# jkrueger/phosphorus_mk2

Hardware: AMD Instinct MI355X
Metric: Mrays/sec (primary+secondary) (higher is better)
Workload: dtype f32; 1 GPU; Soup(100000, seed 1234) 1280x720 256 spp depth 9 pps 1, 1 emissive quad, Lambert 0.73 (BASELINE.json configs[1]); tiles=32x32, tile (tx, ty) -> rank (tx + 3 ty) % n_gpus, film_collective=none, frames_in_flight=1, hbm_bytes_per_rank=41566904552, film_finite=True

## Files before the change

### phosphorus_mk2_amd/csrc/kernels.hip

```cpp
#include "kernels.h"

#include <algorithm>
#include <cstddef>
#include <cstdlib>

namespace phx {

#define PHX_BLOCK 256
#ifndef PHX_PERM_LUT
#define PHX_PERM_LUT 1
#endif
#ifndef PHX_COUNT
#define PHX_COUNT 0
#endif
#ifndef PHX_SHADE_TIMING
#define PHX_SHADE_TIMING 0
#endif
#ifndef PHX_SHADE_PREFETCH
#define PHX_SHADE_PREFETCH 2
#endif

__device__ __forceinline__ uint32_t f2u(float f) { return __float_as_uint(f); }
__device__ __forceinline__ float u2f(uint32_t u) { return __uint_as_float(u); }

#ifndef PHX_SHADE_BLOCK_D
#define PHX_SHADE_BLOCK_D 1024
#endif
#ifndef PHX_SHADE_BLOCK_G
#define PHX_SHADE_BLOCK_G 512
#endif
#ifndef PHX_SHADE_WAVES_G
#define PHX_SHADE_WAVES_G 4
#endif
template <int SHADE_BLOCK>
__device__ __forceinline__ void block_append2(bool want_a, uint32_t* counter_a, bool want_b, uint32_t* counter_b, uint32_t* lds ,
                                              uint32_t& at_a, uint32_t& at_b, unsigned long long* probe = nullptr ) {
  static_assert(SHADE_BLOCK >= 128 && SHADE_BLOCK % 64 == 0, "block_append2: wave 0 sums queue A, wave 1 queue B");
  const uint32_t lane = __lane_id(), wave = threadIdx.x >> 6, nwaves = SHADE_BLOCK >> 6;
  const unsigned long long mask_a = __ballot(want_a), mask_b = __ballot(want_b);
  uint32_t* cnt_a = lds; uint32_t* cnt_b = lds + nwaves + 1;
  if (lane == 0) { cnt_a[wave] = (uint32_t)__popcll(mask_a); cnt_b[wave] = (uint32_t)__popcll(mask_b); }
  __syncthreads();
  if (lane == 0 && wave < 2) {
    uint32_t* cnt = wave == 0 ? cnt_a : cnt_b;
    uint32_t total = 0;
#pragma nounroll
    for (uint32_t w = 0; w < nwaves; ++w) { const uint32_t c = cnt[w]; cnt[w] = total; total += c; }
#if PHX_SHADE_TIMING
    const long long ta_ = clock64();
#endif
    cnt[nwaves] = total ? atomicAdd(wave == 0 ? counter_a : counter_b, total) : 0u;
#if PHX_SHADE_TIMING
    static_assert(offsetof(DevStats, tri_pending_lane_iters) == offsetof(DevStats, idle_lane_iters) + sizeof(unsigned long long), "probe[0] / probe[1] are DevStats::idle_lane_iters / tri_pending_lane_iters");
    if (probe) { asm volatile("s_waitcnt vmcnt(0)" ::: "memory"); atomicAdd(&probe[0], (unsigned long long)(clock64() - ta_)); atomicAdd(&probe[1], 1ull); }
#endif
  }
  __syncthreads();
  const unsigned long long below = (1ull << lane) - 1ull;
  at_a = cnt_a[nwaves] + cnt_a[wave] + (uint32_t)__popcll(mask_a & below);
  at_b = cnt_b[nwaves] + cnt_b[wave] + (uint32_t)__popcll(mask_b & below);
}

template <bool LENS>
__device__ __forceinline__ void camera_ray(const DevScene& sc, const PassBuffers& pb, uint32_t path, uint32_t sample0, v3& p, v3& w) {
  const uint32_t pix = path / pb.num_samples, s = path - pix * pb.num_samples;
  const uint32_t xy = pb.pix_xy[pix];
  const float sx = (float)(xy & 0xffffu), sy = (float)(xy >> 16);
  const float2 jit = pb.jitter[sample0 + s];
  const float ndcy = 0.5f - (-0.5f + sy) * sc.stepy;
  const float ndcx = (-0.5f + sx) * sc.stepx - 0.5f;
  v3 d(jit.x, jit.y, -1.0f);
  d.x = (ndcx + d.x * sc.stepx) * sc.ratio * sc.zoom;
  d.y = (ndcy + d.y * sc.stepy) * sc.zoom;
  const float ool = 1.0f / sqrtf(sdot(d, d));
  d = v3(d.x * ool, d.y * ool, d.z * ool);
  const float* M = sc.cam_m;
  if constexpr (LENS) {
    const uint32_t key = path_key(pb.seed, (xy >> 16) * sc.width + (xy & 0xffffu), sample0 + s);
    const float ux = draw_f32(key, DIM_LENS_U), uy = draw_f32(key, DIM_LENS_V);
    const float c2 = (float)(2.0f / M_PI), c4 = (float)(4.0f / M_PI);
    const bool x_gt_y = fabsf(ux) > fabsf(uy);
    const float r = x_gt_y ? uy : ux;
    const float theta1 = c4 * (uy / ux), theta2 = c2 - c4 * (ux / uy);
    const sincosf_t sc_t = sincosf_(x_gt_y ? theta2 : theta1);
    const float lx = (r * sc_t.c) * sc.aperture_radius, ly = (r * sc_t.s) * sc.aperture_radius;
    const float ft = fabsf(sc.focal_distance / d.z);
    d = v3(d.x * ft - lx, d.y * ft - ly, d.z * ft - 0.0f);
    const float ool2 = 1.0f / sqrtf(sdot(d, d));
    d = v3(d.x * ool2, d.y * ool2, d.z * ool2);
    { float t = lx * M[0]; t = fmaf(ly, M[4], t); t = fmaf(0.0f, M[8], t); p.x = t + M[12]; }
    { float t = lx * M[1]; t = fmaf(ly, M[5], t); t = fmaf(0.0f, M[9], t); p.y = t + M[13]; }
    { float t = lx * M[2]; t = fmaf(ly, M[6], t); t = fmaf(0.0f, M[10], t); p.z = t + M[14]; }
  } else {
  { float t = 0.0f * M[0]; t = fmaf(0.0f, M[4], t); t = fmaf(0.0f, M[8], t); p.x = t + M[12]; }
  { float t = 0.0f * M[1]; t = fmaf(0.0f, M[5], t); t = fmaf(0.0f, M[9], t); p.y = t + M[13]; }
  { float t = 0.0f * M[2]; t = fmaf(0.0f, M[6], t); t = fmaf(0.0f, M[10], t); p.z = t + M[14]; }
  }
  { float t = d.x * M[0]; t = fmaf(d.y, M[4], t); w.x = fmaf(d.z, M[8], t); }
  { float t = d.x * M[1]; t = fmaf(d.y, M[5], t); w.y = fmaf(d.z, M[9], t); }
  { float t = d.x * M[2]; t = fmaf(d.y, M[6], t); w.z = fmaf(d.z, M[10], t); }
}

__device__ __forceinline__ void zero_cursors(uint32_t* counters) {
#pragma unroll
  for (uint32_t k = 0; k < 2u * CNT_SEGS; ++k) counters[CNT_CURSOR + k * CNT_STRIDE] = 0;
}
__global__ void k_begin_pass(PassBuffers pb, uint32_t num_samples) {
  const uint32_t npaths = pb.num_pixels * num_samples;
  pb.counters[0] = npaths; pb.counters[CNT_STRIDE] = 0; pb.counters[CNT_SHADOW] = 0; pb.counters[CNT_SHADOW + CNT_STRIDE] = 0;
  zero_cursors(pb.counters);
  atomicAdd(&pb.stats->camera_samples, (unsigned long long)npaths);
}

template <int LEVELS>
struct LdsStack {
  uint2* base;
  int sp;
  __device__ __forceinline__ void push(uint32_t b, uint32_t h) { base[sp * PHX_BLOCK] = make_uint2(b, h); ++sp; }
  __device__ __forceinline__ void pop(uint32_t& b, uint32_t& h) { --sp; const uint2 e = base[sp * PHX_BLOCK]; b = e.x; h = e.y; }
  __device__ __forceinline__ bool empty() const { return sp == 0; }
};

#ifndef PHX_STEPS_PER_REFILL
#define PHX_STEPS_PER_REFILL 1
#endif
#ifndef PHX_WG_CHUNKS
#define PHX_WG_CHUNKS 16u
#endif
#ifndef PHX_XCD_SEGMENTS
#define PHX_XCD_SEGMENTS 1
#endif
#ifndef PHX_SPILL_FROM_LEVELS
#define PHX_SPILL_FROM_LEVELS 10u
#endif
#ifndef PHX_SPILL_LDS_LEVELS
#define PHX_SPILL_LDS_LEVELS 7u
#endif
#ifndef PHX_STACK_PACKED
#define PHX_STACK_PACKED 1
#endif
#ifndef PHX_PROBE_VALU
#define PHX_PROBE_VALU 0
#endif
#ifndef PHX_PROBE_VMEM
#define PHX_PROBE_VMEM 0
#endif
#ifndef PHX_PROBE_VMEM_DWORD
#define PHX_PROBE_VMEM_DWORD 0
#endif
#define PHX_UNI(x) ((uint32_t)__builtin_amdgcn_readfirstlane((int)(x)))
#ifndef PHX_TRACE_WATCHDOG
#define PHX_TRACE_WATCHDOG (1u << 22)
#endif
struct DynQueue {
  uint32_t n0, n1, c0, c1;
  uint32_t r0, r1;
  uint32_t num_waves;
  uint32_t* cursor;
};
template <int BLOCK, bool SPILL , bool PACKED >
__device__ __forceinline__ void trace_stream(const DevScene& sc, const PassBuffers& pb, int q,
                                             uint32_t* cursor , uint2* stack_base, uint8_t* stack_valid , uint32_t lds_levels,
                                             uint2* spill_base , uint32_t refill_min,
                                             const uint4* __restrict__ top , uint32_t ntop,
                                             const DynQueue dq, const uint8_t* __restrict__ perm_lut) {
  const uint32_t lane = __lane_id();
  bool active = false, any = false;
  uint32_t phase = 0;
  RayCtx r; r.o = v3(0.f); r.d = v3(0.f); r.idx = r.idy = r.idz = 0.f; r.oct_inv = 0;
  float tbest = 0.f, hu = 0.f, hv = 0.f;
  uint32_t htri = 0xffffffffu, hprim = 0, idx = 0, ng_base = 0, ng_hits = 0, path = 0;
  constexpr uint32_t TG_PENDING = 0xff00u;
  uint32_t tg_base = 0, tg = 0, tq_base = 0, tq = 0;
  int sp = 0;
  const float4* __restrict__ ro = pb.ro[q];
  const float4* __restrict__ rd = pb.rd[q];
  uint32_t dlo = 0, dhi = 0;
#if PHX_COUNT
  uint32_t cnt_lds[2] = {0, 0}, cnt_mem[2] = {0, 0}, cnt_tri[2] = {0, 0};
  uint32_t cnt_iter = 0, cnt_nb = 0, cnt_tb = 0, cnt_refill = 0;
  uint32_t cnt_idle = 0, cnt_pend = 0;
  uint32_t cnt_push[8] = {0, 0, 0, 0, 0, 0, 0, 0};
  uint32_t cnt_pairs = 0, cnt_pairs_hist[8] = {0, 0, 0, 0, 0, 0, 0, 0};
#endif
  uint32_t guard = 0;
  for (;;) {
    if (++guard > PHX_TRACE_WATCHDOG) { if (lane == 0) atomicAdd(&pb.stats->watchdog, 1ull); break; }
    const unsigned long long idle = __ballot(!active);
    if (phase < 2u && (uint32_t)__popcll(idle) >= refill_min) {
#if PHX_COUNT
      ++cnt_refill;
#endif
      const uint32_t leader = (uint32_t)__ffsll((long long)idle) - 1u;
      uint32_t hi, base;
      {
        if (dlo >= dhi) {
          const uint32_t c = phase == 0u ? dq.c0 : dq.c1, qn = phase == 0u ? dq.n0 : dq.n1;
          uint32_t got_lo = 0, got_hi = 0, st = 1;
          if (lane == leader) {
            unsigned long long* pack = reinterpret_cast<unsigned long long*>(cursor) + phase;
            uint32_t* fetching = cursor + 4 + phase; uint32_t* done = cursor + 6 + phase;
            const unsigned long long old = __hip_atomic_fetch_add(pack, (unsigned long long)c, __ATOMIC_RELAXED, __HIP_MEMORY_SCOPE_WORKGROUP);
            const uint32_t s0 = (uint32_t)old, e0 = (uint32_t)(old >> 32);
            if (s0 < e0) { got_lo = s0; got_hi = min(s0 + c, e0); st = 0; }
            else if (__hip_atomic_load(done, __ATOMIC_RELAXED, __HIP_MEMORY_SCOPE_WORKGROUP)) st = 2;
            else if (atomicCAS(fetching, 0u, 1u) == 0u) {
              __builtin_amdgcn_fence(__ATOMIC_ACQUIRE, "workgroup");
              const unsigned long long cur = __hip_atomic_load(pack, __ATOMIC_RELAXED, __HIP_MEMORY_SCOPE_WORKGROUP);
              if ((uint32_t)cur < (uint32_t)(cur >> 32)) st = 1;
              else if (__hip_atomic_load(done, __ATOMIC_RELAXED, __HIP_MEMORY_SCOPE_WORKGROUP)) st = 2;
              else {
                const uint32_t cwg = phase == 0u ? dq.r0 : dq.r1;
#if PHX_XCD_SEGMENTS
                uint32_t nb = qn, seg_end = qn, sgm = cursor[8 + phase];
                for (uint32_t tries = 0; tries < CNT_SEGS; ++tries, sgm = (sgm + 1u) & (CNT_SEGS - 1u)) {
                  const uint32_t lo_s = (uint32_t)((unsigned long long)qn * sgm / CNT_SEGS), hi_s = (uint32_t)((unsigned long long)qn * (sgm + 1u) / CNT_SEGS);
                  const uint32_t homes = (gridDim.x + CNT_SEGS - 1u - sgm) / CNT_SEGS;
                  const unsigned long long at = (unsigned long long)lo_s + (unsigned long long)homes * cwg + atomicAdd(&dq.cursor[(phase * CNT_SEGS + sgm) * CNT_STRIDE], cwg);
                  if (at < hi_s) { nb = (uint32_t)at; seg_end = hi_s; break; }
                }
                cursor[8 + phase] = sgm;
                if (nb >= seg_end) { __hip_atomic_store(done, 1u, __ATOMIC_RELAXED, __HIP_MEMORY_SCOPE_WORKGROUP); st = 2; }
                else {
                  const uint32_t end = min(nb + cwg, seg_end);
#else
                const uint32_t nb = atomicAdd(&dq.cursor[phase * CNT_SEGS * CNT_STRIDE], cwg) + gridDim.x * cwg;
                if (nb >= qn) { __hip_atomic_store(done, 1u, __ATOMIC_RELAXED, __HIP_MEMORY_SCOPE_WORKGROUP); st = 2; }
                else {
                  const uint32_t end = min(nb + cwg, qn);
#endif
                  got_lo = nb; got_hi = min(nb + c, end); st = 0;
                  __hip_atomic_store(pack, (unsigned long long)(nb + c) | ((unsigned long long)end << 32), __ATOMIC_RELAXED, __HIP_MEMORY_SCOPE_WORKGROUP);
                }
              }
              __builtin_amdgcn_fence(__ATOMIC_RELEASE, "workgroup");
              __hip_atomic_store(fetching, 0u, __ATOMIC_RELAXED, __HIP_MEMORY_SCOPE_WORKGROUP);
            }
          }
          st = (uint32_t)__builtin_amdgcn_readfirstlane((int)__shfl((int)st, (int)leader));
          if (st == 2u) {
            phase = PHX_UNI(phase + 1u);
            if (phase < 2u || __ballot(active) != 0ull) { if (phase < 2u) continue; } else break;
          } else if (st == 0u) {
            dlo = (uint32_t)__builtin_amdgcn_readfirstlane((int)__shfl((int)got_lo, (int)leader));
            dhi = (uint32_t)__builtin_amdgcn_readfirstlane((int)__shfl((int)got_hi, (int)leader));
          } else if (__ballot(active) == 0ull) { __builtin_amdgcn_s_sleep(4); continue; }
        }
        if (phase >= 2u) { hi = 0; base = 0; }
        else {
          const uint32_t take = PHX_UNI(min((uint32_t)__popcll(idle), dhi - dlo));
          base = dlo; hi = dlo + take; dlo = PHX_UNI(dlo + take);
        }
      }
      if (!active) {
        const uint32_t l5 = lane & 31u, below = (1u << l5) - 1u, ilo = (uint32_t)idle, ihi = (uint32_t)(idle >> 32);
        const uint32_t my = base + (uint32_t)__popc(ilo & below) + (uint32_t)__popc(ihi & below) + (lane >= 32u ? ((ilo >> l5) & 1u) : 0u);
        if (my < hi) {
          {
            float4 a, b;
            if (phase == 0u) { a = pb.so[my]; b = pb.sd[my]; } else { a = ro[my]; b = rd[my]; }
            r = make_ray_ctx(v3(a.x, a.y, a.z), v3(b.x, b.y, b.z));
            tbest = phase == 0u ? b.w : FLT_MAX; path = f2u(a.w);
          }
          hu = 0.f; hv = 0.f; htri = 0xffffffffu; hprim = 0; idx = my;
          ng_base = 0; ng_hits = 0x80000000u; tg = 0; tq = 0; sp = 0;
          any = phase == 0u;
          active = true;
        }
      }
      if (phase < 2u && __ballot(active) == 0ull) continue;
    }
    if (!__ballot(active)) break;
#if PHX_COUNT
    ++cnt_iter;
    cnt_idle += (uint32_t)__popcll(__ballot(!active));
#endif
    const bool node_ok = active && ng_hits > 0x00ffffffu && (any ? !(tg & TG_PENDING) : tq == 0u);
#if PHX_COUNT
    if (__ballot(node_ok)) ++cnt_nb;
    cnt_pend += (uint32_t)__popcll(__ballot(active && !node_ok && (tg & TG_PENDING)));
#endif
    if (node_ok) {
      const uint32_t bit = 31u - (uint32_t)__clz((int)ng_hits);
      const uint32_t rest = ng_hits & ~(1u << bit);
      if (rest > 0x00ffffffu) {
#if PHX_COUNT
        ++cnt_push[sp < 7 ? sp : 7];
#endif
        if (!SPILL || (uint32_t)sp < lds_levels) {
          if constexpr (PACKED) {
            reinterpret_cast<uint32_t*>(stack_base)[sp * BLOCK] = (ng_base & 0x00ffffffu) | (rest & 0xff000000u);
            stack_valid[((uint32_t)sp >> 2) * (BLOCK * 4u) + ((uint32_t)sp & 3u)] = (uint8_t)rest;
          } else stack_base[sp * BLOCK] = make_uint2(ng_base, rest);
        }
        else spill_base[(size_t)((uint32_t)sp - lds_levels) * sc.spill_stride] = make_uint2(ng_base, rest);
        ++sp;
      }
      const uint32_t slot = (bit - 24u) ^ r.oct_inv;
      const uint32_t ni = ng_base + (uint32_t)__popc(ng_hits & 0xffu & ~(0xffffffffu << slot));
      uint32_t w[16];
#if PHX_COUNT
      if (ni < ntop) ++cnt_lds[any ? 1 : 0]; else ++cnt_mem[any ? 1 : 0];
#endif
      const bool in_lds = ni < ntop;
      {
        const uint4* s4 = top + (in_lds ? ni : 0u) * (PHX_NODE_LDS_BYTES / 16u);
#pragma unroll
        for (int k = 0; k < 4; ++k) { const uint4 v = s4[k]; w[4 * k] = v.x; w[4 * k + 1] = v.y; w[4 * k + 2] = v.z; w[4 * k + 3] = v.w; }
      }
      if (!in_lds) {
        const uint4* s4 = reinterpret_cast<const uint4*>(sc.pool) + (size_t)ni * 4u;
#pragma unroll
        for (int k = 0; k < 4; ++k) { const uint4 v = s4[k]; w[4 * k] = v.x; w[4 * k + 1] = v.y; w[4 * k + 2] = v.z; w[4 * k + 3] = v.w; }
      }
#if PHX_PROBE_VMEM
      if (!in_lds) {
        const uint4* s4 = reinterpret_cast<const uint4*>(sc.pool) + (size_t)(ni ^ 1u) * 4u;
#pragma unroll
        for (int k = 0; k < PHX_PROBE_VMEM; ++k) {
#if PHX_PROBE_VMEM_DWORD
          w[2] ^= s4[k].x & (refill_min >> 31);
#else
          const uint4 v = s4[k]; w[2] ^= (v.x ^ v.y ^ v.z ^ v.w) & (refill_min >> 31);
#endif
        }
      }
#endif
#if PHX_PERM_LUT
      uint32_t hm = node_hitmask(w, sc.grid, r, tbest, [&](uint32_t m) { return (uint32_t)perm_lut[(r.oct_inv << 8) | m]; });
#else
      uint32_t hm = node_hitmask(w, sc.grid, r, tbest);
#endif
#if PHX_PROBE_VALU
      {
        float x = tbest;
#pragma unroll
        for (int k = 0; k < PHX_PROBE_VALU; ++k) x = __builtin_fmaf(x, 0.99999f, 1.0e-3f);
        hm ^= f2u(x) & (refill_min >> 31);
      }
#endif
      ng_base = w[3];
      ng_hits = hm & 0xff0000ffu;
      const uint32_t tnew = (hm >> 8) & TG_PENDING;
      if (tnew) {
        const uint32_t g = (hm & 0xffu) | tnew;
        if (!(tg & TG_PENDING)) { tg_base = w[3]; tg = g; }
        else { tq_base = w[3]; tq = g; }
      }
    }
    const bool tpend = active && (tg & TG_PENDING);
#if PHX_COUNT
    if (__ballot(tpend)) {
      ++cnt_tb;
      const uint32_t mine = active ? (uint32_t)__popc((tg >> 8) & 0xffu) + (uint32_t)__popc((tq >> 8) & 0xffu) : 0u;
      uint32_t pairs = 0;
      for (uint32_t b = 0; b < 5u; ++b) pairs += (uint32_t)__popcll(__ballot((mine >> b) & 1u)) << b;
      cnt_pairs += pairs;
      ++cnt_pairs_hist[pairs <= 8u ? 0 : pairs <= 16u ? 1 : pairs <= 24u ? 2 : pairs <= 32u ? 3 : pairs <= 48u ? 4 : pairs <= 64u ? 5 : pairs <= 96u ? 6 : 7];
    }
#endif
    if (tpend) {
      const uint32_t k = 23u - (uint32_t)__clz((int)(tg & TG_PENDING));
      tg &= ~(0x100u << k);
      const uint32_t ti = tg_base + (uint32_t)__popc(tg & 0xffu & ~(0xffffffffu << k));
      const uint4* t4 = reinterpret_cast<const uint4*>(sc.pool) + (size_t)ti * 4u;
      const uint4 t0 = t4[0], t1 = t4[1], t2 = t4[2];
      TriRec T;
      T.v0x = u2f(t0.x); T.v0y = u2f(t0.y); T.v0z = u2f(t0.z); T.e0x = u2f(t0.w);
      T.e0y = u2f(t1.x); T.e0z = u2f(t1.y); T.e1x = u2f(t1.z); T.e1y = u2f(t1.w);
      T.e1z = u2f(t2.x); T.prim = t2.y;
      float us, vs, ds;
#if PHX_COUNT
      ++cnt_tri[any ? 1 : 0];
#endif
      if (mt_intersect(T, r.o, r.d, tbest, hprim, us, vs, ds)) {
        tbest = ds; hu = us; hv = vs; htri = ti; hprim = T.prim;
        if (any) active = false;
      }
      if (!(tg & TG_PENDING) && tq != 0u) { tg_base = tq_base; tg = tq; tq = 0u; }
    }
    if (active && ng_hits <= 0x00ffffffu) {
      if (sp == 0) {
        if (!(tg & TG_PENDING)) {
          if (any) {
            const float4 cc = pb.sc[idx];
            float4 rr = pb.pr[path];
            rr.x += cc.x; rr.y += cc.y; rr.z += cc.z;
            pb.pr[path] = rr;
          } else {
            pb.hit[idx] = make_float4(tbest, hu, hv, u2f(htri));
          }
          active = false;
        }
      } else {
        --sp;
        uint2 e;
        if (!SPILL || (uint32_t)sp < lds_levels) {
          if constexpr (PACKED) {
            const uint32_t word = reinterpret_cast<uint32_t*>(stack_base)[sp * BLOCK];
            const uint32_t vb = stack_valid[((uint32_t)sp >> 2) * (BLOCK * 4u) + ((uint32_t)sp & 3u)];
            e = make_uint2(word & 0x00ffffffu, (word & 0xff000000u) | vb);
          } else e = stack_base[sp * BLOCK];
        }
        else e = spill_base[(size_t)((uint32_t)sp - lds_levels) * sc.spill_stride];
        ng_base = e.x; ng_hits = e.y;
      }
    }
  }
#if PHX_COUNT
  for (int k = 0; k < 2; ++k) {
    atomicAdd(&pb.stats->node_visits_lds[k], (unsigned long long)cnt_lds[k]);
    atomicAdd(&pb.stats->node_visits_mem[k], (unsigned long long)cnt_mem[k]);
    atomicAdd(&pb.stats->tri_tests[k], (unsigned long long)cnt_tri[k]);
  }
  for (int k = 0; k < 8; ++k) if (cnt_push[k]) atomicAdd(&pb.stats->stack_pushes[k], (unsigned long long)cnt_push[k]);
  if (lane == 0) {
    atomicAdd(&pb.stats->tri_block_execs, (unsigned long long)cnt_tb);
    atomicAdd(&pb.stats->wave_iters, (unsigned long long)cnt_iter);
    atomicAdd(&pb.stats->node_block_execs, (unsigned long long)cnt_nb);
    atomicAdd(&pb.stats->refills, (unsigned long long)cnt_refill);
    atomicAdd(&pb.stats->idle_lane_iters, (unsigned long long)cnt_idle);
    atomicAdd(&pb.stats->tri_pending_lane_iters, (unsigned long long)cnt_pend);
    atomicAdd(&pb.stats->tri_pairs_pending, (unsigned long long)cnt_pairs);
    for (int k = 0; k < 8; ++k) if (cnt_pairs_hist[k]) atomicAdd(&pb.stats->tri_pairs_hist[k], (unsigned long long)cnt_pairs_hist[k]);
  }
#endif
}

template <int BLOCK, bool SPILL = false, bool PACKED = false>
__global__ void __launch_bounds__(BLOCK, 8) k_trace(DevScene sc, PassBuffers pb, int q, int sq, int do_closest, int do_shadow, uint32_t refill_min,
                                                 uint32_t ntop, uint32_t levels, uint32_t min_chunks, uint32_t target_chunks) {
  extern __shared__ uint4 smem[];
  uint4* top = smem;
  uint2* stack = reinterpret_cast<uint2*>(smem + ntop * (PHX_NODE_LDS_BYTES / 16u));
  uint32_t* stack_words = reinterpret_cast<uint32_t*>(stack);
  uint32_t* valid_rows = stack_words + levels * BLOCK;
  uint32_t* cursor = PACKED ? valid_rows + ((levels + 3u) >> 2) * BLOCK : reinterpret_cast<uint32_t*>(stack + levels * BLOCK);
  uint8_t* perm_lut = reinterpret_cast<uint8_t*>(cursor + 12);
  const uint32_t n_closest = do_closest ? pb.counters[q * CNT_STRIDE] : 0u;
  const uint32_t n_shadow = do_shadow ? pb.counters[CNT_SHADOW + sq * CNT_STRIDE] : 0u;
  if (blockIdx.x == 0 && threadIdx.x == 0) {
    if (do_closest) { pb.counters[(q ^ 1) * CNT_STRIDE] = 0; pb.counters[CNT_SHADOW + (sq ^ 1) * CNT_STRIDE] = 0; }
    if (n_closest) atomicAdd(&pb.stats->rays_closest, (unsigned long long)n_closest);
    if (n_shadow) atomicAdd(&pb.stats->rays_shadow, (unsigned long long)n_shadow);
    if (do_closest && pb.qlen_out) { __hip_atomic_store(pb.qlen_out, n_closest, __ATOMIC_RELAXED, __HIP_MEMORY_SCOPE_SYSTEM); }
  }
  if (n_shadow == 0u && n_closest == 0u) return;
  DynQueue dq{};
  dq.n0 = n_shadow; dq.n1 = n_closest;
  dq.num_waves = gridDim.x * (BLOCK / 64);
  dq.cursor = pb.counters + CNT_CURSOR;
  auto chunk_of = [&](uint32_t n) { return min(max((n / (dq.num_waves * max(min_chunks, 1u)) + 63u) & ~63u, 64u), target_chunks * 64u); };
  dq.c0 = chunk_of(n_shadow); dq.c1 = chunk_of(n_closest);
  auto range_of = [&](uint32_t n, uint32_t c) { return c * min(max(n / (gridDim.x * c * 4u), 1u), PHX_WG_CHUNKS); };
  dq.r0 = range_of(n_shadow, dq.c0); dq.r1 = range_of(n_closest, dq.c1);
  if (threadIdx.x == 0) {
    unsigned long long* pack = reinterpret_cast<unsigned long long*>(cursor);
    for (uint32_t p = 0; p < 2u; ++p) {
      const uint32_t cwg = p == 0u ? dq.r0 : dq.r1, qn = p == 0u ? n_shadow : n_closest;
#if PHX_XCD_SEGMENTS
      const uint32_t sgm = blockIdx.x & (CNT_SEGS - 1u), kth = blockIdx.x / CNT_SEGS;
      const uint32_t lo_s = (uint32_t)((unsigned long long)qn * sgm / CNT_SEGS), hi_s = (uint32_t)((unsigned long long)qn * (sgm + 1u) / CNT_SEGS);
      const uint32_t lo = (uint32_t)min((unsigned long long)lo_s + (unsigned long long)kth * cwg, (unsigned long long)hi_s), hi = min(lo + cwg, hi_s);
      cursor[8 + p] = sgm;
#else
      const uint32_t lo = min(blockIdx.x * cwg, qn), hi = min(lo + cwg, qn);
#endif
      pack[p] = (unsigned long long)lo | ((unsigned long long)hi << 32);
      cursor[4 + p] = 0u; cursor[6 + p] = 0u;
    }
  }
  const uint4* g4 = reinterpret_cast<const uint4*>(sc.pool);
  for (uint32_t i = threadIdx.x; i < ntop * 4u; i += BLOCK) top[(i >> 2) * (PHX_NODE_LDS_BYTES / 16u) + (i & 3u)] = g4[i];
#if PHX_PERM_LUT
  for (uint32_t i = threadIdx.x; i < 2048u; i += BLOCK) perm_lut[i] = (uint8_t)perm_xor8(i & 0xffu, i >> 8);
#endif
  __syncthreads();
  if constexpr (PACKED)
    trace_stream<BLOCK, SPILL, true>(sc, pb, q, cursor, reinterpret_cast<uint2*>(stack_words + threadIdx.x), reinterpret_cast<uint8_t*>(valid_rows + threadIdx.x), levels,
                                     sc.stack_spill + (size_t)blockIdx.x * BLOCK + threadIdx.x, refill_min, top, ntop, dq, perm_lut);
  else
    trace_stream<BLOCK, SPILL, false>(sc, pb, q, cursor, stack + threadIdx.x, nullptr, levels, sc.stack_spill + (size_t)blockIdx.x * BLOCK + threadIdx.x,
                                      refill_min, top, ntop, dq, perm_lut);
}

template <bool ANY>
__global__ void __launch_bounds__(PHX_BLOCK) k_trace_rays(DevScene sc, uint32_t n, const float4* ro, const float4* rd, float4* hit) {
  extern __shared__ uint2 ray_stack[];
  const uint32_t i = blockIdx.x * PHX_BLOCK + threadIdx.x;
  if (i >= n) return;
  const float4 a = ro[i], b = rd[i];
  LdsStack<0> st{ray_stack + threadIdx.x, 0};
  Hit h;
  traverse8<ANY>(sc.pool, sc.grid, v3(a.x, a.y, a.z), v3(b.x, b.y, b.z), b.w, h, st);
  hit[i] = make_float4(h.t, h.u, h.v, u2f(h.tri == 0xffffffffu ? 0xffffffffu : sc.tris[h.tri].prim));
}

template <bool MAX>
__device__ __forceinline__ float wave_reduce_f(float x) {
#define PHX_DPP_STEP(ctrl, rows) { const float t = __builtin_bit_cast(float, __builtin_amdgcn_update_dpp(__builtin_bit_cast(int, x), __builtin_bit_cast(int, x), ctrl, rows, 0xf, false)); x = MAX ? fmaxf(x, t) : fminf(x, t); }
  PHX_DPP_STEP(0x111, 0xf) PHX_DPP_STEP(0x112, 0xf) PHX_DPP_STEP(0x114, 0xf) PHX_DPP_STEP(0x118, 0xf)
  PHX_DPP_STEP(0x142, 0xa) PHX_DPP_STEP(0x143, 0xc)
#undef PHX_DPP_STEP
  return __builtin_bit_cast(float, __builtin_amdgcn_readlane(__builtin_bit_cast(int, x), 63));
}
__device__ __forceinline__ float wave_min_f(float x) { return wave_reduce_f<false>(x); }
__device__ __forceinline__ float wave_max_f(float x) { return wave_reduce_f<true>(x); }
struct PacketBounds { float s[3], kn[3], kf[3], bmin[3], bmax[3]; };
__device__ __forceinline__ void packet_axis(PacketBounds& B, int a, float o_lo, float o_hi, float ia_lo, float ia_hi ,
                                            bool down ) {
  const float omin = wave_min_f(o_lo), omax = wave_max_f(o_hi);
  B.bmin[a] = wave_min_f(ia_lo); B.bmax[a] = wave_max_f(ia_hi);
  B.s[a] = down ? -1.0f : 1.0f;
  B.kn[a] = down ? omin : -omax;
  B.kf[a] = down ? omax : -omin;
}
typedef unsigned int phx_u4 __attribute__((ext_vector_type(4)));
typedef const __attribute__((address_space(4))) phx_u4* phx_const_u4p;
__device__ __forceinline__ uint32_t packet_node_hit8(const uint32_t* w, const SceneGrid& g, const PacketBounds& B, uint32_t oct_inv, float tmax_wave, uint32_t& valid) {
  float px, py, pz;
  node_origin_decode(w[0], w[1], g, px, py, pz, valid);
  const uint32_t e = w[2];
  const float sx = u32_as_f32((e & 0xffu) << 23), sy = u32_as_f32(((e >> 8) & 0xffu) << 23), sz = u32_as_f32(((e >> 16) & 0xffu) << 23);
  const uint32_t sh = (__lane_id() & 7u) * 8u;
  auto plane = [&](int row) { return (float)((uint32_t)((((unsigned long long)w[row + 1] << 32) | (unsigned long long)w[row]) >> sh) & 0xffu); };
  const float lox = fmaf(plane(4), sx, px), hix = fmaf(plane(10), sx, px);
  const float loy = fmaf(plane(6), sy, py), hiy = fmaf(plane(12), sy, py);
  const float loz = fmaf(plane(8), sz, pz), hiz = fmaf(plane(14), sz, pz);
  const bool nx = !(oct_inv & 4u), ny = !(oct_inv & 2u), nz = !(oct_inv & 1u);
  const float anx = fmaf(B.s[0], nx ? hix : lox, B.kn[0]), afx = fmaf(B.s[0], nx ? lox : hix, B.kf[0]);
  const float any_ = fmaf(B.s[1], ny ? hiy : loy, B.kn[1]), afy = fmaf(B.s[1], ny ? loy : hiy, B.kf[1]);
  const float anz = fmaf(B.s[2], nz ? hiz : loz, B.kn[2]), afz = fmaf(B.s[2], nz ? loz : hiz, B.kf[2]);
  const float tnx = anx * (anx >= 0.0f ? B.bmin[0] : B.bmax[0]), tfx = afx * (afx >= 0.0f ? B.bmax[0] : B.bmin[0]);
  const float tny = any_ * (any_ >= 0.0f ? B.bmin[1] : B.bmax[1]), tfy = afy * (afy >= 0.0f ? B.bmax[1] : B.bmin[1]);
  const float tnz = anz * (anz >= 0.0f ? B.bmin[2] : B.bmax[2]), tfz = afz * (afz >= 0.0f ? B.bmax[2] : B.bmin[2]);
  float tn = fmaxf(fmaxf(tnx, tny), tnz), tf = fminf(fminf(tfx, tfy), tfz);
  const float pad = 1.52587890625e-05f;
  tn = tn - fabsf(tn) * pad; tf = tf + fabsf(tf) * pad;
  const bool hit = tn <= tf && tf >= 0.0f && tn <= tmax_wave;
  return (uint32_t)__ballot(hit) & 0xffu & valid;
}

#define PHX_PRIMARY_BLOCK 256
#ifndef PHX_PRIMARY_WAVES
#define PHX_PRIMARY_WAVES 5
#endif
template <int RPL, bool LENS = false >
__global__ void __launch_bounds__(PHX_PRIMARY_BLOCK) __attribute__((amdgpu_waves_per_eu(PHX_PRIMARY_WAVES, 8))) k_trace_primary(DevScene sc, PassBuffers pb, uint32_t npaths, uint32_t sample0, int q, int sq) {
  extern __shared__ uint2 primary_lds[];
  uint2* lane_stacks = primary_lds + (PHX_PRIMARY_BLOCK / 64) * PHX_MAX_BVH_DEPTH;
  if (blockIdx.x == 0 && threadIdx.x == 0) {
    pb.counters[(q ^ 1) * CNT_STRIDE] = 0; pb.counters[CNT_SHADOW + (sq ^ 1) * CNT_STRIDE] = 0;
    atomicAdd(&pb.stats->rays_closest, (unsigned long long)npaths);
  }
  const uint32_t lane = __lane_id(), wave = threadIdx.x >> 6;
  const uint32_t base = (blockIdx.x * (PHX_PRIMARY_BLOCK / 64) + wave) * (64u * RPL);
  if (base >= npaths) return;
  uint32_t idx[RPL];
  RayCtx r[RPL];
  float tbest[RPL], hu[RPL], hv[RPL];
  uint32_t htri[RPL], hprim[RPL];
  bool mixed = false;
#pragma unroll
  for (int k = 0; k < RPL; ++k) {
    idx[k] = base + 64u * k + lane;
    v3 co, cd;
    camera_ray<LENS>(sc, pb, min(idx[k], npaths - 1u), sample0, co, cd);
    r[k] = make_ray_ctx(co, cd);
    tbest[k] = FLT_MAX; hu[k] = 0.0f; hv[k] = 0.0f; htri[k] = 0xffffffffu; hprim[k] = 0;
  }
  const uint32_t oct = PHX_UNI(r[0].oct_inv);
#pragma unroll
  for (int k = 0; k < RPL; ++k) mixed = mixed || r[k].oct_inv != oct;
  if (__ballot(mixed) != 0ull) {
#pragma unroll
    for (int k = 0; k < RPL; ++k) {
      LdsStack<0> st{lane_stacks + threadIdx.x, 0};
      Hit h;
      if constexpr (LENS) { const float chk = (r[k].o.x + r[k].o.y + r[k].o.z) + (r[k].d.x + r[k].d.y + r[k].d.z); if (!(fabsf(chk) <= FLT_MAX)) continue; }
      traverse8<false>(sc.pool, sc.grid, r[k].o, r[k].d, FLT_MAX, h, st);
      tbest[k] = h.t; hu[k] = h.u; hv[k] = h.v; htri[k] = h.tri;
    }
#if PHX_COUNT
    if (lane == 0) { atomicAdd(&pb.stats->primary_packets, 1ull); atomicAdd(&pb.stats->primary_fallbacks, 1ull); }
#endif
  } else {
    PacketBounds B;
    {
      v3 olo = r[0].o, ohi = r[0].o, ilo(fabsf(r[0].idx), fabsf(r[0].idy), fabsf(r[0].idz)), ihi = ilo;
#pragma unroll
      for (int k = 1; k < RPL; ++k) {
        olo = v3(fminf(olo.x, r[k].o.x), fminf(olo.y, r[k].o.y), fminf(olo.z, r[k].o.z)); ohi = v3(fmaxf(ohi.x, r[k].o.x), fmaxf(ohi.y, r[k].o.y), fmaxf(ohi.z, r[k].o.z));
        const v3 ia(fabsf(r[k].idx), fabsf(r[k].idy), fabsf(r[k].idz));
        ilo = v3(fminf(ilo.x, ia.x), fminf(ilo.y, ia.y), fminf(ilo.z, ia.z)); ihi = v3(fmaxf(ihi.x, ia.x), fmaxf(ihi.y, ia.y), fmaxf(ihi.z, ia.z));
      }
      packet_axis(B, 0, olo.x, ohi.x, ilo.x, ihi.x, !(oct & 4u)); packet_axis(B, 1, olo.y, ohi.y, ilo.y, ihi.y, !(oct & 2u)); packet_axis(B, 2, olo.z, ohi.z, ilo.z, ihi.z, !(oct & 1u));
    }
    float tmax_wave = FLT_MAX;
    uint32_t ng_base = 0, ng_hits = 0x80000000u;
    uint32_t sp = 0, guard = 0;
#if PHX_COUNT
    uint32_t cnt_nodes = 0, cnt_tris = 0, cnt_lanes = 0;
#endif
    uint2* stack = primary_lds + wave * PHX_MAX_BVH_DEPTH;
    for (;;) {
      if (++guard > PHX_TRACE_WATCHDOG) { if (lane == 0) atomicAdd(&pb.stats->watchdog, 1ull); break; }
      const uint32_t bit = 31u - (uint32_t)__clz((int)ng_hits);
      const uint32_t rest = ng_hits & ~(1u << bit);
      if (rest > 0x00ffffffu) { if (lane == 0) stack[sp] = make_uint2(ng_base, rest); ++sp; }
      const uint32_t slot = (bit - 24u) ^ oct;
      const uint32_t ni = PHX_UNI(ng_base + (uint32_t)__popc(ng_hits & 0xffu & ~(0xffffffffu << slot)));
      uint32_t w[16];
      {
        const phx_const_u4p s4 = (phx_const_u4p)(sc.pool) + (size_t)ni * 4u;
#pragma unroll
        for (int k = 0; k < 4; ++k) { const phx_u4 v = s4[k]; w[4 * k] = v.x; w[4 * k + 1] = v.y; w[4 * k + 2] = v.z; w[4 * k + 3] = v.w; }
      }
      uint32_t valid;
#if PHX_COUNT
      ++cnt_nodes;
#endif
      const uint32_t hit8 = packet_node_hit8(w, sc.grid, B, oct, tmax_wave, valid);
      const uint32_t imask = w[2] >> 24;
      ng_base = PHX_UNI(w[3]);
      ng_hits = PHX_UNI((perm_xor8(hit8 & imask, oct) << 24) | valid);
      uint32_t th = PHX_UNI(hit8 & ~imask);
      while (th != 0u) {
        const uint32_t k = 31u - (uint32_t)__clz((int)th);
        th &= ~(1u << k);
        const uint32_t ti = PHX_UNI(ng_base + (uint32_t)__popc(valid & ~(0xffffffffu << k)));
        const phx_const_u4p t4 = (phx_const_u4p)(sc.pool) + (size_t)ti * 4u;
        const phx_u4 t0 = t4[0], t1 = t4[1], t2 = t4[2];
        TriRec T;
        T.v0x = u2f(t0.x); T.v0y = u2f(t0.y); T.v0z = u2f(t0.z); T.e0x = u2f(t0.w);
        T.e0y = u2f(t1.x); T.e0z = u2f(t1.y); T.e1x = u2f(t1.z); T.e1y = u2f(t1.w);
        T.e1z = u2f(t2.x); T.prim = t2.y;
        bool any_better = false;
        float tworst = 0.0f;
#pragma unroll
        for (int m = 0; m < RPL; ++m) {
          float us, vs, ds;
          const bool better = mt_intersect(T, r[m].o, r[m].d, tbest[m], hprim[m], us, vs, ds);
          if (better) { tbest[m] = ds; hu[m] = us; hv[m] = vs; htri[m] = ti; hprim[m] = T.prim; }
          any_better = any_better || better;
          tworst = fmaxf(tworst, tbest[m]);
        }
#if PHX_COUNT
        ++cnt_tris; cnt_lanes += (uint32_t)__popcll(__ballot(any_better));
#endif
        if (__ballot(any_better) != 0ull) tmax_wave = wave_max_f(tworst);
      }
      if (ng_hits <= 0x00ffffffu) {
        if (sp == 0u) break;
        --sp;
        const uint2 e = stack[sp];
        ng_base = PHX_UNI(e.x); ng_hits = PHX_UNI(e.y);
      }
    }
#if PHX_COUNT
    if (lane == 0) {
      atomicAdd(&pb.stats->primary_packets, 1ull);
      atomicAdd(&pb.stats->primary_node_tests, (unsigned long long)cnt_nodes);
      atomicAdd(&pb.stats->primary_tri_tests, (unsigned long long)cnt_tris);
      atomicAdd(&pb.stats->primary_tri_lanes_hit, (unsigned long long)cnt_lanes);
    }
#endif
  }
#pragma unroll
  for (int k = 0; k < RPL; ++k)
    if (idx[k] < npaths) pb.hit[idx[k]] = make_float4(tbest[k], hu[k], hv[k], u2f(htri[k]));
}

__device__ __forceinline__ v3 shading_normal(const DevScene& sc, uint32_t elem , bool smooth, const v3& e0, const v3& e1, float u, float v) {
  if (smooth) {
    const float w = 1 - u - v;
    const float* pn = sc.elem_normals + 9 * (size_t)elem;
    const v3 n0(pn[0], pn[1], pn[2]), n1(pn[3], pn[4], pn[5]), n2(pn[6], pn[7], pn[8]);
    return normalize_inplace(w * n0 + u * n1 + v * n2);
  }
  return normalize_inplace(cross(e0, e1));
}
struct VertexNormals { v3 n0, n1, n2; };
__device__ __forceinline__ VertexNormals request_vertex_normals(const DevScene& sc, uint32_t elem) {
  VertexNormals N{v3(0.0f), v3(0.0f), v3(0.0f)};
  if (sc.elem_normals) {
    const float* pn = sc.elem_normals + 9 * (size_t)elem;
    N.n0 = v3(pn[0], pn[1], pn[2]); N.n1 = v3(pn[3], pn[4], pn[5]); N.n2 = v3(pn[6], pn[7], pn[8]);
  }
  return N;
}
__device__ __forceinline__ v3 shading_normal(const VertexNormals& N, bool smooth, const v3& geometric , float u, float v) {
  if (smooth) { const float w = 1 - u - v; return normalize_inplace(w * N.n0 + u * N.n1 + v * N.n2); }
  return geometric;
}

struct CornerUVs { float2 a, b, c; };
__device__ __forceinline__ CornerUVs request_corner_uvs(const float2* elem_uv, uint32_t elem) {
  const float2* p = elem_uv + 3 * (size_t)elem;
  return CornerUVs{p[0], p[1], p[2]};
}
__device__ __forceinline__ float2 hit_st(const CornerUVs& C, float u, float v) {
  const float w = (1 - u) - v;
  return make_float2((w * C.a.x + u * C.b.x) + v * C.c.x, (w * C.a.y + u * C.b.y) + v * C.c.y);
}

__device__ __forceinline__ float luminance(const v3& c) {
  return (float)0.212671 * c.x + (float)0.715160 * c.y + (float)0.072169 * c.z;
}

template <int MATS ,
          bool FIRST , bool LENS = false >
__global__ void __launch_bounds__(PHX_SHADE_BLOCK_D) __attribute__((amdgpu_waves_per_eu(4, 8))) k_shade(DevScene sc, PassBuffers pb, int q, int sq, uint32_t sample0) {
  static_assert(MATS == 1 || MATS == 2, "general closures: k_shade_g");
  constexpr bool DIFFUSE_ONLY = true;
  constexpr int MAXL = MATS == 2 ? 1 : 8;
  constexpr int PHX_SHADE_BLOCK = PHX_SHADE_BLOCK_D;
  __shared__ uint32_t lds_cnt[2 * ((PHX_SHADE_BLOCK >> 6) + 1)];
  if (pb.stats->watchdog | pb.stats->ring_watchdog) return;
  const uint32_t count = pb.counters[q * CNT_STRIDE];
  const uint32_t i = blockIdx.x * PHX_SHADE_BLOCK + threadIdx.x;
  if (i == 0) zero_cursors(pb.counters);
  if (blockIdx.x * PHX_SHADE_BLOCK >= count) return;
  const bool live = i < count;
  bool alive = false, want_shadow = false, masked = false;
  uint32_t path = 0, next_specular = 0;
  v3 nxt_o, nxt_d, sh_o, sh_d, contrib, nxt_beta;
  uint32_t nxt_depth = 0, key = 0;
  float sh_t = 0.0f;
  if (live) {
    float4 a, b, bd;
    const float4 h = pb.hit[i];
    if (FIRST) {
      v3 co, cd;
      camera_ray<LENS>(sc, pb, i, sample0, co, cd);
      a = make_float4(co.x, co.y, co.z, u2f(i)); b = make_float4(cd.x, cd.y, cd.z, FLT_MAX);
      bd = make_float4(1.0f, 1.0f, 1.0f, u2f(0u));
    } else {
      a = pb.ro[q][i]; b = pb.rd[q][i]; bd = pb.qs[q][i];
    }
    const uint32_t pbits = f2u(a.w);
    path = pbits & 0x7fffffffu;
    const bool specular = (pbits >> 31) != 0;
    v3 beta(bd.x, bd.y, bd.z);
    v3 add_e(0.0f); bool add_rad = false;
    const bool beta_finite = isfinite(bd.x) && isfinite(bd.y) && isfinite(bd.z);
    uint32_t depth = f2u(bd.w);
    if (FIRST) {
      const uint32_t pix = path / pb.num_samples, s = path - pix * pb.num_samples;
      const uint32_t xy = pb.pix_xy[pix];
      key = path_key(pb.seed, (xy >> 16) * sc.width + (xy & 0xffffu), sample0 + s);
    } else {
      key = f2u(b.w);
    }
    const uint32_t tri = f2u(h.w);
    const v3 o(a.x, a.y, a.z), d(b.x, b.y, b.z);
    if (tri != 0xffffffffu) {
      const float4 S = sc.elem_shade[tri];
      const uint32_t pm = f2u(S.w);
      const v3 p = o + d * h.x;
      const v3 wo = -d;
      const v3 n = (pm >> 31) != 0 ? shading_normal(sc, tri, true, v3(0.0f), v3(0.0f), h.y, h.z) : v3(S.x, S.y, S.z);
      const DevMaterial* mp = &sc.materials[pm & 0x7fffffffu];
      DevMaterial mh;
      if (MATS == 2) {
        const DevMatLite ml = sc.mat_lite[pm & 0x7fffffffu];
        mh.num_lobes = ml.lobes_flags & 0xffu; mh.lobes[0].flags = ml.lobes_flags >> 8; mh.lobes[0].type = L_DIFFUSE;
        mh.lobes[0].wx = ml.wx; mh.lobes[0].wy = ml.wy; mh.lobes[0].wz = ml.wz;
        mh.ex = ml.ex; mh.ey = ml.ey; mh.ez = ml.ez; mh.sheen_L5 = 0.0f;
        mp = &mh;
      }
      const DevMaterial& m = *mp;
      if (pb.pn && (FIRST || depth == 0)) pb.pn[path] = make_float4(n.x, n.y, n.z, 1.0f);
      const v3 e(m.ex, m.ey, m.ez);
      if (depth == 0 || specular) { add_e = e; add_rad = true; }
      {
        const uint32_t b0 = depth * DIMS_PER_STEP;
        const float pick = draw_f32(key, b0 + DIM_LIGHT_PICK), lu = draw_f32(key, b0 + DIM_LIGHT_U), lv = draw_f32(key, b0 + DIM_LIGHT_V);
        const float nlf = (float)sc.num_lights;
        uint32_t l = (uint32_t)floorf(pick * nlf);
        if (l > sc.num_lights - 1) l = sc.num_lights - 1;
        const DevLight L = sc.lights[l];
        const float numf = (float)L.num_tris;
        uint32_t ti = (uint32_t)floorf(lu * numf);
        if (ti > L.num_tris - 1) ti = L.num_tris - 1;
        const float remapped = fminf(lu * numf - (float)ti, 1.0f - FLT_EPSILON);
// ... 958 lines not shown
```

Before: 9767 Mrays/s.

## Defer finished-ray writes to refill and recompute stack pointers to cut registers

Finished rays no longer write their results inside the traversal loop. They set a flag and write at the next refill, where the lanes are already divergent, which takes the stores off the hot node/triangle path. Stack and spill pointers are now rebuilt on the fly from threadIdx.x, passed through an opaque asm so they are not held as 64-bit VGPRs for the whole loop. The chunk and range values are marked wave-uniform, and optional timing instrumentation is added. The aims are lower register pressure and less divergence, at the cost of some extra address arithmetic and delayed writes.

```diff
diff --git a/phosphorus_mk2_amd/csrc/kernels.hip b/phosphorus_mk2_amd/csrc/kernels.hip
--- a/phosphorus_mk2_amd/csrc/kernels.hip
+++ b/phosphorus_mk2_amd/csrc/kernels.hip
@@ -152,6 +152,44 @@
 #ifndef PHX_TRACE_WATCHDOG
 #define PHX_TRACE_WATCHDOG (1u << 22)
 #endif
+#ifndef PHX_TRACE_TIMING
+#define PHX_TRACE_TIMING 0
+#endif
+#ifndef PHX_DEFER_FINISH
+#define PHX_DEFER_FINISH 1
+#endif
+#if PHX_TRACE_TIMING
+#if PHX_COUNT
+#error "PHX_TRACE_TIMING reuses DevStats fields of the count build"
+#endif
+#define PHX_TT_DECL uint32_t tt_acc[6] = {0, 0, 0, 0, 0, 0}, tt_iters = 0, tt_fin = 0; long long tt_t = clock64();
+#define PHX_TT(n) { asm volatile("s_waitcnt vmcnt(0) lgkmcnt(0)" ::: "memory"); const long long now_ = clock64(); tt_acc[n] += (uint32_t)(now_ - tt_t); tt_t = now_; }
+#define PHX_TT_DUMP(closest) { \
+    if (lane == 0) { \
+      unsigned long long* d_ = (closest) ? pb.stats->tri_pairs_hist : pb.stats->stack_pushes; \
+      for (int k_ = 0; k_ < 6; ++k_) atomicAdd(d_ + k_, (unsigned long long)tt_acc[k_]); \
+      atomicAdd(d_ + 6, (unsigned long long)tt_iters); atomicAdd(d_ + 7, (unsigned long long)tt_fin); \
+    } \
+    for (int k_ = 0; k_ < 6; ++k_) tt_acc[k_] = 0; \
+    tt_iters = 0; tt_fin = 0; }
+#else
+#define PHX_TT_DECL
+#define PHX_TT(n)
+#define PHX_TT_DUMP(closest)
+#endif
+#define PHX_FLUSH_LANE() { \
+    if (any) { \
+      const float4 cc_ = pb.sc[idx]; \
+      float4 rr_ = pb.pr[path]; \
+      rr_.x += cc_.x; rr_.y += cc_.y; rr_.z += cc_.z; \
+      pb.pr[path] = rr_; \
+    } else pb.hit[idx] = make_float4(tbest, hu, hv, u2f(htri)); }
+#define PHX_STACK_MINE() \
+  uint2* stack_base = stack_base_; uint8_t* stack_valid = stack_valid_; uint32_t spill_col = spill_col_; \
+  if constexpr (SPILL) { \
+    uint32_t t_ = threadIdx.x; asm volatile("" : "+v"(t_)); \
+    stack_base = PACKED ? reinterpret_cast<uint2*>(reinterpret_cast<uint32_t*>(stack_base_) + t_) : stack_base_ + t_; \
+    stack_valid = stack_valid_ + 4u * t_; spill_col = spill_col_ + t_; }
 struct DynQueue {
   uint32_t n0, n1, c0, c1;
   uint32_t r0, r1;
@@ -160,8 +198,8 @@
 };
 template <int BLOCK, bool SPILL , bool PACKED >
 __device__ __forceinline__ void trace_stream(const DevScene& sc, const PassBuffers& pb, int q,
-                                             uint32_t* cursor , uint2* stack_base, uint8_t* stack_valid , uint32_t lds_levels,
-                                             uint2* spill_base , uint32_t refill_min,
+                                             uint32_t* cursor , uint2* stack_base_, uint8_t* stack_valid_ , uint32_t lds_levels,
+                                             uint32_t spill_col_ , uint32_t refill_min,
                                              const uint4* __restrict__ top , uint32_t ntop,
                                              const DynQueue dq, const uint8_t* __restrict__ perm_lut) {
   const uint32_t lane = __lane_id();
@@ -184,6 +222,8 @@
   uint32_t cnt_pairs = 0, cnt_pairs_hist[8] = {0, 0, 0, 0, 0, 0, 0, 0};
 #endif
   uint32_t guard = 0;
+  bool flush = false;
+  PHX_TT_DECL
   for (;;) {
     if (++guard > PHX_TRACE_WATCHDOG) { if (lane == 0) atomicAdd(&pb.stats->watchdog, 1ull); break; }
     const unsigned long long idle = __ballot(!active);
@@ -239,6 +279,9 @@
           }
           st = (uint32_t)__builtin_amdgcn_readfirstlane((int)__shfl((int)st, (int)leader));
           if (st == 2u) {
+#if PHX_TRACE_TIMING
+            if (phase == 0u) PHX_TT_DUMP(false)
+#endif
             phase = PHX_UNI(phase + 1u);
             if (phase < 2u || __ballot(active) != 0ull) { if (phase < 2u) continue; } else break;
           } else if (st == 0u) {
@@ -252,25 +295,33 @@
           base = dlo; hi = dlo + take; dlo = PHX_UNI(dlo + take);
         }
       }
+      PHX_TT(0)
+#if PHX_TRACE_TIMING
+      if (flush) { PHX_FLUSH_LANE() flush = false; }
+      PHX_TT(5)
+#endif
       if (!active) {
         const uint32_t l5 = lane & 31u, below = (1u << l5) - 1u, ilo = (uint32_t)idle, ihi = (uint32_t)(idle >> 32);
         const uint32_t my = base + (uint32_t)__popc(ilo & below) + (uint32_t)__popc(ihi & below) + (lane >= 32u ? ((ilo >> l5) & 1u) : 0u);
+        if (flush) { PHX_FLUSH_LANE() flush = false; }
         if (my < hi) {
-          {
-            float4 a, b;
-            if (phase == 0u) { a = pb.so[my]; b = pb.sd[my]; } else { a = ro[my]; b = rd[my]; }
-            r = make_ray_ctx(v3(a.x, a.y, a.z), v3(b.x, b.y, b.z));
-            tbest = phase == 0u ? b.w : FLT_MAX; path = f2u(a.w);
-          }
+          float4 a, b;
+          if (phase == 0u) { a = pb.so[my]; b = pb.sd[my]; } else { a = ro[my]; b = rd[my]; }
+          r = make_ray_ctx(v3(a.x, a.y, a.z), v3(b.x, b.y, b.z));
+          tbest = phase == 0u ? b.w : FLT_MAX; path = f2u(a.w);
           hu = 0.f; hv = 0.f; htri = 0xffffffffu; hprim = 0; idx = my;
           ng_base = 0; ng_hits = 0x80000000u; tg = 0; tq = 0; sp = 0;
           any = phase == 0u;
           active = true;
         }
       }
+      PHX_TT(1)
       if (phase < 2u && __ballot(active) == 0ull) continue;
     }
     if (!__ballot(active)) break;
+#if PHX_TRACE_TIMING
+    ++tt_iters;
+#endif
 #if PHX_COUNT
     ++cnt_iter;
     cnt_idle += (uint32_t)__popcll(__ballot(!active));
@@ -280,6 +331,7 @@
     if (__ballot(node_ok)) ++cnt_nb;
     cnt_pend += (uint32_t)__popcll(__ballot(active && !node_ok && (tg & TG_PENDING)));
 #endif
+    uint32_t w[16];
     if (node_ok) {
       const uint32_t bit = 31u - (uint32_t)__clz((int)ng_hits);
       const uint32_t rest = ng_hits & ~(1u << bit);
@@ -287,18 +339,18 @@
 #if PHX_COUNT
         ++cnt_push[sp < 7 ? sp : 7];
 #endif
+        PHX_STACK_MINE()
         if (!SPILL || (uint32_t)sp < lds_levels) {
           if constexpr (PACKED) {
             reinterpret_cast<uint32_t*>(stack_base)[sp * BLOCK] = (ng_base & 0x00ffffffu) | (rest & 0xff000000u);
             stack_valid[((uint32_t)sp >> 2) * (BLOCK * 4u) + ((uint32_t)sp & 3u)] = (uint8_t)rest;
           } else stack_base[sp * BLOCK] = make_uint2(ng_base, rest);
         }
-        else spill_base[(size_t)((uint32_t)sp - lds_levels) * sc.spill_stride] = make_uint2(ng_base, rest);
+        else sc.stack_spill[((uint32_t)sp - lds_levels) * sc.spill_stride + spill_col] = make_uint2(ng_base, rest);
         ++sp;
       }
       const uint32_t slot = (bit - 24u) ^ r.oct_inv;
       const uint32_t ni = ng_base + (uint32_t)__popc(ng_hits & 0xffu & ~(0xffffffffu << slot));
-      uint32_t w[16];
 #if PHX_COUNT
       if (ni < ntop) ++cnt_lds[any ? 1 : 0]; else ++cnt_mem[any ? 1 : 0];
 #endif
@@ -325,6 +377,11 @@
 #endif
         }
       }
+#endif
+#if PHX_TRACE_TIMING
+    }
+    PHX_TT(2)
+    if (node_ok) {
 #endif
 #if PHX_PERM_LUT
       uint32_t hm = node_hitmask(w, sc.grid, r, tbest, [&](uint32_t m) { return (uint32_t)perm_lut[(r.oct_inv << 8) | m]; });
@@ -348,6 +405,7 @@
         else { tq_base = w[3]; tq = g; }
       }
     }
+    PHX_TT(3)
     const bool tpend = active && (tg & TG_PENDING);
 #if PHX_COUNT
     if (__ballot(tpend)) {
@@ -379,22 +437,24 @@
       }
       if (!(tg & TG_PENDING) && tq != 0u) { tg_base = tq_base; tg = tq; tq = 0u; }
     }
+    PHX_TT(4)
+#if PHX_TRACE_TIMING
+    tt_fin += (uint32_t)__popcll(__ballot(active && ng_hits <= 0x00ffffffu && sp == 0 && !(tg & TG_PENDING)));
+#endif
     if (active && ng_hits <= 0x00ffffffu) {
       if (sp == 0) {
         if (!(tg & TG_PENDING)) {
-          if (any) {
-            const float4 cc = pb.sc[idx];
-            float4 rr = pb.pr[path];
-            rr.x += cc.x; rr.y += cc.y; rr.z += cc.z;
-            pb.pr[path] = rr;
-          } else {
-            pb.hit[idx] = make_float4(tbest, hu, hv, u2f(htri));
-          }
+#if PHX_DEFER_FINISH
+          flush = true;
+#else
+          PHX_FLUSH_LANE()
+#endif
           active = false;
         }
       } else {
         --sp;
         uint2 e;
+        PHX_STACK_MINE()
         if (!SPILL || (uint32_t)sp < lds_levels) {
           if constexpr (PACKED) {
             const uint32_t word = reinterpret_cast<uint32_t*>(stack_base)[sp * BLOCK];
@@ -402,11 +462,15 @@
             e = make_uint2(word & 0x00ffffffu, (word & 0xff000000u) | vb);
           } else e = stack_base[sp * BLOCK];
         }
-        else e = spill_base[(size_t)((uint32_t)sp - lds_levels) * sc.spill_stride];
+        else e = sc.stack_spill[((uint32_t)sp - lds_levels) * sc.spill_stride + spill_col];
         ng_base = e.x; ng_hits = e.y;
       }
     }
-  }
+    PHX_TT(5)
+  }
+  if (flush) PHX_FLUSH_LANE()
+  PHX_TT(5)
+  PHX_TT_DUMP(phase != 0u)
 #if PHX_COUNT
   for (int k = 0; k < 2; ++k) {
     atomicAdd(&pb.stats->node_visits_lds[k], (unsigned long long)cnt_lds[k]);
@@ -451,9 +515,9 @@
   dq.num_waves = gridDim.x * (BLOCK / 64);
   dq.cursor = pb.counters + CNT_CURSOR;
   auto chunk_of = [&](uint32_t n) { return min(max((n / (dq.num_waves * max(min_chunks, 1u)) + 63u) & ~63u, 64u), target_chunks * 64u); };
-  dq.c0 = chunk_of(n_shadow); dq.c1 = chunk_of(n_closest);
+  dq.c0 = PHX_UNI(chunk_of(n_shadow)); dq.c1 = PHX_UNI(chunk_of(n_closest));
   auto range_of = [&](uint32_t n, uint32_t c) { return c * min(max(n / (gridDim.x * c * 4u), 1u), PHX_WG_CHUNKS); };
-  dq.r0 = range_of(n_shadow, dq.c0); dq.r1 = range_of(n_closest, dq.c1);
+  dq.r0 = PHX_UNI(range_of(n_shadow, dq.c0)); dq.r1 = PHX_UNI(range_of(n_closest, dq.c1));
   if (threadIdx.x == 0) {
     unsigned long long* pack = reinterpret_cast<unsigned long long*>(cursor);
     for (uint32_t p = 0; p < 2u; ++p) {
@@ -477,10 +541,10 @@
 #endif
   __syncthreads();
   if constexpr (PACKED)
-    trace_stream<BLOCK, SPILL, true>(sc, pb, q, cursor, reinterpret_cast<uint2*>(stack_words + threadIdx.x), reinterpret_cast<uint8_t*>(valid_rows + threadIdx.x), levels,
-                                     sc.stack_spill + (size_t)blockIdx.x * BLOCK + threadIdx.x, refill_min, top, ntop, dq, perm_lut);
+    trace_stream<BLOCK, SPILL, true>(sc, pb, q, cursor, reinterpret_cast<uint2*>(stack_words + (SPILL ? 0u : threadIdx.x)), reinterpret_cast<uint8_t*>(valid_rows + (SPILL ? 0u : threadIdx.x)), levels,
+                                     blockIdx.x * BLOCK, refill_min, top, ntop, dq, perm_lut);
   else
-    trace_stream<BLOCK, SPILL, false>(sc, pb, q, cursor, stack + threadIdx.x, nullptr, levels, sc.stack_spill + (size_t)blockIdx.x * BLOCK + threadIdx.x,
+    trace_stream<BLOCK, SPILL, false>(sc, pb, q, cursor, stack + (SPILL ? 0u : threadIdx.x), nullptr, levels, blockIdx.x * BLOCK,
                                       refill_min, top, ntop, dq, perm_lut);
 }
 
```

Measured after the change: 9678 Mrays/s. No clear change (-0.9%).
